# leotimus/recommender-tensorflow

Measured on AMD Instinct MI355X. Metric: examples/sec DeepFM batch=65536 (full train step), higher is better.
Workload: dtype f32 (MLP GEMM operands: fp16 hi+lo split, 3 products, fp32 accumulate)

## Files before the change

include/mi355x_rec.h:

```cpp
#ifndef MI355X_REC_H
#define MI355X_REC_H

#include <stddef.h>
#include <stdint.h>

#ifdef __cplusplus
extern "C" {
#endif

typedef void* mi_stream_t;

enum mi_status {
  MI_OK = 0,
  MI_ERR_INVALID = -1,
  MI_ERR_UNSUPPORTED = -2,
  MI_ERR_LAUNCH = -3,
  MI_ERR_WORKSPACE = -4
};

int32_t mi_abi_version(void);
const char* mi_last_error(void);
const char* mi_build_info(void);

typedef struct mi_step_state {
// ... 100 lines not shown
  float lr_t;
  float decay, momentum;
  float lr_power, l1, l2;
} mi_opt_hparams;

int32_t mi_axpy(float* y, const float* x, int64_t n, float alpha, mi_stream_t stream);

int32_t mi_dense_apply(float* param, float* slot0, float* slot1, const float* grad, int64_t n,
                       const mi_opt_hparams* hp, mi_stream_t stream);

int32_t mi_sparse_apply(float* table, float* t_slot0, float* t_slot1, float* lin_w, float* l_slot0,
                        float* l_slot1, int32_t* last_step, const int32_t* uniq_rows,
                        const int32_t* seg_start, const int32_t* sorted_entry,
                        const int32_t* num_uniq, int64_t n_max, const float* d_rows,
                        const float* d_lin, int32_t E, int32_t step, const mi_opt_hparams* hp,
                        int32_t lin_stride, int64_t table_stride, int64_t grad_stride, mi_stream_t stream);

int32_t mi_sparse_apply_fused(float* table, float* t_slot0, float* t_slot1, float* lin_w, float* l_slot0,
                              float* l_slot1, int32_t* last_step, const int32_t* uniq_rows,
                              const int32_t* seg_start, const int32_t* sorted_entry, const int32_t* num_uniq,
                              int64_t n_max, const float* d_concat, int64_t ld_dconcat, const float* sumv,
                              const float* d_logit_fm, const float* d_logit_lin, int32_t F, int32_t E,
                              int32_t step, const mi_opt_hparams* hp, int32_t lin_stride, int64_t table_stride, mi_stream_t stream);

enum mi_catchup_flags { MI_CATCHUP_DEFER_SLOTS = 1, MI_CATCHUP_BOUNDED = 2, MI_CATCHUP_KEEP_STAMPS = 4, MI_CATCHUP_LOCAL_ORDER = 8 };
int32_t mi_catchup_local_chunk_rows(void);
int32_t mi_catchup_bounded_runs(float beta1, float beta2, float epsilon);
int32_t mi_catchup_local_plan(int64_t n_max, int64_t num_uniq, int64_t* plan);
int32_t mi_catchup_gap_keys(const int32_t* uniq_rows, const int32_t* num_uniq, const int32_t* last_step, int64_t n_max,
                            int32_t step_to, int32_t* keys, int32_t lin_stride, mi_stream_t stream);

int32_t mi_catchup_rows_by_gap(const int32_t* uniq_rows, const int32_t* num_uniq, const int32_t* last_step, int64_t n_max,
                               int32_t step_to, int32_t lin_stride, int32_t* rows_out, void* workspace,
                               size_t workspace_bytes, mi_stream_t stream);


int32_t mi_selftest_sqrt(uint32_t first_bits, int64_t count, uint64_t* mismatches, mi_stream_t stream);

int32_t mi_selftest_div(float d, uint32_t first_bits, int64_t count, uint64_t* out, mi_stream_t stream);

int32_t mi_sparse_catchup(float* table, float* t_m, float* t_v, float* lin_w, float* l_m, float* l_v,
                          int32_t* last_step, const int32_t* uniq_rows, const int32_t* num_uniq,
                          int64_t n_max, int32_t E, int32_t step_to, const float* lr_table,
                          float beta1, float beta2, float epsilon, int32_t flags, int32_t lin_stride,
                          int64_t table_stride, mi_stream_t stream);

// ... 266 lines not shown
```

recommender-tensorflow_amd/csrc/optim.hip:

```cpp
#include "common.h"
#include "optim_rules.h"
#include <algorithm>

namespace {

constexpr int kBlock = 256;

__global__ __launch_bounds__(kBlock) void dense_apply_k(float* __restrict__ w, float* __restrict__ s0,
                                                        float* __restrict__ s1,
                                                        const float* __restrict__ g, int64_t n,
                                                        Hp h, const mi_step_state_t* __restrict__ st) {
  if (st) h.lr_t = st->lr_t;
  const int64_t stride = static_cast<int64_t>(gridDim.x) * kBlock;
  for (int64_t i = static_cast<int64_t>(blockIdx.x) * kBlock + threadIdx.x; i < n; i += stride) {
    float wv = w[i], a = s0 ? s0[i] : 0.f, b = s1 ? s1[i] : 0.f;
    dense_rule(h, wv, a, b, g[i]);
    w[i] = wv;
    if (s0) s0[i] = a;
    if (s1) s1[i] = b;
  }
}

typedef float f32x4_t __attribute__((ext_vector_type(4)));
__device__ __forceinline__ float4 ld4_nt(const float* p) {
// ... 5 lines not shown
  __builtin_nontemporal_store(x, reinterpret_cast<f32x4_t*>(p));
}

struct FusedGrad {
  const float* d_concat; int64_t ldd; const float* sumv; const float* dlf; const float* dll; int F;
  int64_t b0;
};

constexpr int kLongSeg = 48;
constexpr int kRun = 1;

struct ApplyArgs {
  float* table; float* t0; float* t1;
  float* lin_w; float* l0; float* l1;
  int32_t* last_step;
  const int32_t* uniq_rows; const int32_t* seg_start; const int32_t* sorted_entry; const int32_t* num_uniq;
  const float* d_rows; const float* d_lin;
  int E, step;
  float* out_rows; float* out_lin; int u_begin, u_count;
  int ls;
  const mi_step_state_t* st;
  int64_t ts;
  int64_t gs, gls, os, ols;
};

template <bool FUSED>
__device__ __forceinline__ void seg_accumulate(const ApplyArgs& a, const FusedGrad& fg, int k_beg, int k_end, int l,
                                               bool lane_on, const float4& w, float4& g, float& gl) {
  const int E = a.E;
  for (int k = k_beg; k < k_end; ++k) {
    const int64_t e = a.sorted_entry[k];
    if constexpr (FUSED) {
      const int64_t bg = e / fg.F;
      const int f = static_cast<int>(e - bg * fg.F);
      const int64_t b = bg - fg.b0;
      if (a.table && lane_on) {
        float4 v = make_float4(0.f, 0.f, 0.f, 0.f);
        if (fg.d_concat) v = ld4(fg.d_concat + b * fg.ldd + static_cast<int64_t>(f) * E + 4 * l);
        if (fg.dlf) {
          const float gf = fg.dlf[b];
          if (fg.sumv) {
            const float4 sv = ld4(fg.sumv + b * E + 4 * l);
            v.x += gf * (sv.x - w.x); v.y += gf * (sv.y - w.y);
            v.z += gf * (sv.z - w.z); v.w += gf * (sv.w - w.w);
          } else {
            v.x -= gf * w.x; v.y -= gf * w.y; v.z -= gf * w.z; v.w -= gf * w.w;
          }
// ... 58 lines not shown
      for (int j = 0; j < missed; ++j) { s0 = s0 * h.beta1; s1 = s1 * h.beta2; }
      sparse_rule(h, lw, s0, s1, gl);
      a.lin_w[o] = lw;
      if (a.l0) a.l0[o] = s0;
      if (a.l1) a.l1[o] = s1;
    }
    if (a.last_step) a.last_step[r * a.ls] = a.step;
  }
}

__device__ __forceinline__ void store_row(const ApplyArgs& a, int64_t u, int l, bool lane_on, const float4& g, float gl) {
  if (a.out_rows && lane_on) st4(a.out_rows + u * a.os + 4 * l, g);
  if (a.out_lin && l == 0) a.out_lin[u * a.ols] = gl;
}

template <int LPR, bool FUSED, bool STORE = false>
__global__ __launch_bounds__(kBlock) void sparse_apply_k(ApplyArgs a, Hp h, const FusedGrad fg) {
  if (a.st) { a.step = a.st->step; h.lr_t = a.st->lr_t; }
  int64_t u = (static_cast<int64_t>(blockIdx.x) * kBlock + threadIdx.x) / LPR;
  const int l = threadIdx.x & (LPR - 1);
  if (u >= (STORE ? a.u_count : *a.num_uniq)) return;
  if (STORE) u += a.u_begin;
  const int s_beg = a.seg_start[u], s_end = a.seg_start[u + 1];
  if (s_end - s_beg > kLongSeg) return;
  const int64_t r = STORE ? u : static_cast<int64_t>(a.uniq_rows[u]);
  const bool lane_on = 4 * l < a.E;
  float4 g = make_float4(0.f, 0.f, 0.f, 0.f);
  float gl = 0.f;
  float4 w = make_float4(0.f, 0.f, 0.f, 0.f);
  if (a.table && lane_on && (!STORE || fg.dlf)) w = ld4(a.table + r * a.ts + 4 * l);
  RowState q;
  if constexpr (!STORE) q = load_row_state(a, h, r, l, lane_on);
  seg_accumulate<FUSED>(a, fg, s_beg, s_end, l, lane_on, w, g, gl);
  if constexpr (STORE) store_row(a, u, l, lane_on, g, gl);
  else apply_row(a, h, r, l, lane_on, w, g, gl, q);
}

template <int LPR, bool FUSED, bool STORE = false>
__global__ __launch_bounds__(kBlock) void sparse_apply_long_k(ApplyArgs a, Hp h, const FusedGrad fg) {
  if (a.st) { a.step = a.st->step; h.lr_t = a.st->lr_t; }
  constexpr int G = kBlock / LPR;
  __shared__ int list[kBlock];
  __shared__ int n_list;
  __shared__ float4 part[kBlock];
  __shared__ float part_l[G];
  const int U = STORE ? a.u_count : *a.num_uniq;
  const int ub = STORE ? a.u_begin : 0;
  const int t = threadIdx.x, l = t & (LPR - 1), grp = t / LPR;
  const bool lane_on = 4 * l < a.E;
  const int64_t per_round = static_cast<int64_t>(kBlock) * gridDim.x;
  {
    int any = 0;
    for (int64_t base = 0; base < U; base += per_round) {
      const int64_t u = base + (static_cast<int64_t>(t / kRun) * gridDim.x + blockIdx.x) * kRun + t % kRun;
      if (u < U) any |= (a.seg_start[ub + u + 1] - a.seg_start[ub + u] > kLongSeg) ? 1 : 0;
    }
    if (!__syncthreads_or(any)) return;
  }
  for (int64_t base = 0; base < U; base += per_round) {
    if (t == 0) n_list = 0;
    __syncthreads();
    const int64_t u = base + (static_cast<int64_t>(t / kRun) * gridDim.x + blockIdx.x) * kRun + t % kRun;
    if (u < U && a.seg_start[ub + u + 1] - a.seg_start[ub + u] > kLongSeg) list[atomicAdd(&n_list, 1)] = static_cast<int>(ub + u);
    __syncthreads();
    const int n = n_list;
    for (int j = 0; j < n; ++j) {
      const int uu = list[j];
      const int64_t r = STORE ? static_cast<int64_t>(uu) : static_cast<int64_t>(a.uniq_rows[uu]);
      const int s_beg = a.seg_start[uu], s_end = a.seg_start[uu + 1];
      const int per = (s_end - s_beg + G - 1) / G;
      const int k0 = min(s_end, s_beg + grp * per), k1 = min(s_end, k0 + per);
      float4 g = make_float4(0.f, 0.f, 0.f, 0.f);
      float gl = 0.f;
      float4 w = make_float4(0.f, 0.f, 0.f, 0.f);
      if (a.table && lane_on && (!STORE || fg.dlf)) w = ld4(a.table + r * a.ts + 4 * l);
      seg_accumulate<FUSED>(a, fg, k0, k1, l, lane_on, w, g, gl);
      part[t] = g;
      if (l == 0) part_l[grp] = gl;
      __syncthreads();
      if (grp == 0) {
        g = part[l];
        gl = part_l[0];
#pragma unroll 4
        for (int q = 1; q < G; ++q) {
          const float4 v = part[q * LPR + l];
          g.x += v.x; g.y += v.y; g.z += v.z; g.w += v.w;
          gl += part_l[q];
        }
        if constexpr (STORE) store_row(a, uu, l, lane_on, g, gl);
        else apply_row(a, h, r, l, lane_on, w, g, gl, load_row_state(a, h, r, l, lane_on));
      }
      __syncthreads();
    }
  }
}

__device__ __forceinline__ float sqrt_rn_fixup(float x) {
  float s = __builtin_amdgcn_sqrtf(x);
  const float sm = __uint_as_float(__float_as_uint(s) - 1u), sp = __uint_as_float(__float_as_uint(s) + 1u);
  const float rm = fmaf(-sm, s, x), rp = fmaf(-sp, s, x);
  s = (rm <= 0.f) ? sm : s;
  s = (rp > 0.f) ? sp : s;
  return s;
}
__device__ __forceinline__ float sqrt_rn_inrange(float x) {
  const float r = __builtin_amdgcn_rsqf(x);
  float s = x * r, h = 0.5f * r;
  const float e = fmaf(-h, s, 0.5f);
  h = fmaf(h, e, h);
  s = fmaf(s, e, s);
  const float d = fmaf(-s, s, x);
  return fmaf(d, h, s);
}
__device__ __forceinline__ float div_rn_inrange(float n, float d) {
  float r = __builtin_amdgcn_rcpf(d);
  const float e = fmaf(-d, r, 1.0f);
// ... 474 lines not shown
    default: { constexpr int L = 64; CALL; } break; \
  }

static int32_t check_hp(const char* who, const mi_opt_hparams* hp) {
  if (!hp || hp->kind < MI_OPT_ADAM || hp->kind > MI_OPT_SGD) {
    mi::set_error("%s: bad optimizer kind", who);
    return MI_ERR_INVALID;
  }
  if (hp->kind == MI_OPT_FTRL && hp->lr_power != -0.5f) {
    mi::set_error("%s: Ftrl learning_rate_power %f unsupported (TF default -0.5 only)", who, hp->lr_power);
    return MI_ERR_UNSUPPORTED;
  }
  return MI_OK;
}

__global__ __launch_bounds__(kBlock) void axpy_k(float* __restrict__ y, const float* __restrict__ x, int64_t n, float alpha) {
  const int64_t i = static_cast<int64_t>(blockIdx.x) * kBlock + threadIdx.x;
  if (i < n) y[i] = y[i] + alpha * x[i];
}

unsigned long_grid(int64_t n_max) {
  return static_cast<unsigned>(std::min<int64_t>(1024, mi::ceil_div(n_max, kBlock)));
}

__global__ void step_advance_k(mi_step_state_t* __restrict__ st, const float* __restrict__ lr_table) {
  const int s = st->step + 1;
  st->step = s;
  st->lr_t = lr_table ? lr_table[s] : 0.f;
  st->seed_term = static_cast<uint64_t>(s) * 1000003ull;
}

extern "C" {

int32_t mi_step_advance(mi_step_state_t* device_state, const float* lr_table, mi_stream_t stream) {
  MI_REQUIRE(device_state, "step_advance: null state");
  step_advance_k<<<dim3(1), dim3(1), 0, mi::as_stream(stream)>>>(device_state, lr_table);
  MI_CHECK_LAUNCH("step_advance");
  return MI_OK;
}

int32_t mi_axpy(float* y, const float* x, int64_t n, float alpha, mi_stream_t stream) {
  MI_REQUIRE(n >= 0 && (n == 0 || (x && y)), "axpy: n=%lld", (long long)n);
  if (n == 0) return MI_OK;
  axpy_k<<<dim3((unsigned)mi::ceil_div(n, kBlock)), dim3(kBlock), 0, mi::as_stream(stream)>>>(y, x, n, alpha);
  MI_CHECK_LAUNCH("axpy");
  return MI_OK;
}


int32_t mi_dense_apply(float* param, float* slot0, float* slot1, const float* grad, int64_t n,
                       const mi_opt_hparams* hp, mi_stream_t stream) {
  if (int32_t rc = check_hp("dense_apply", hp)) return rc;
  MI_REQUIRE(n >= 0, "dense_apply: n=%lld", (long long)n);
  if (n == 0) return MI_OK;
  MI_REQUIRE(param && grad, "dense_apply: null buffer");
  MI_REQUIRE(hp->kind == MI_OPT_SGD || slot0, "dense_apply: optimizer needs slot0");
  MI_REQUIRE((hp->kind != MI_OPT_ADAM && hp->kind != MI_OPT_FTRL && hp->kind != MI_OPT_RMSPROP) || slot1,
             "dense_apply: optimizer needs slot1");
  int64_t nb = mi::ceil_div(n, kBlock);
  if (nb > 4096) nb = 4096;
  dense_apply_k<<<dim3((unsigned)nb), dim3(kBlock), 0, mi::as_stream(stream)>>>(param, slot0, slot1, grad, n, make_hp(hp), mi::step_state());
  MI_CHECK_LAUNCH("dense_apply");
  return MI_OK;
}

int32_t mi_sparse_apply(float* table, float* t_slot0, float* t_slot1, float* lin_w, float* l_slot0,
                        float* l_slot1, int32_t* last_step, const int32_t* uniq_rows,
                        const int32_t* seg_start, const int32_t* sorted_entry,
                        const int32_t* num_uniq, int64_t n_max, const float* d_rows,
                        const float* d_lin, int32_t E, int32_t step, const mi_opt_hparams* hp,
                        int32_t lin_stride, int64_t table_stride, int64_t grad_stride, mi_stream_t stream) {
  if (int32_t rc = check_hp("sparse_apply", hp)) return rc;
  MI_REQUIRE(grad_stride == 0 || (grad_stride >= (table ? E : 1) && (!table || (grad_stride & 3) == 0)),
             "sparse_apply: grad_stride=%lld (0 = d_rows E apart and d_lin 1 apart, else one record per entry)", (long long)grad_stride);
  if (!table) table_stride = 0;
  MI_REQUIRE(table_stride == 0 || (table_stride >= E && (table_stride & 3) == 0), "%s: table_stride=%lld (0 = E, else >= E and a multiple of 4)", "sparse_apply", (long long)table_stride);
  const int64_t ts = table_stride ? table_stride : E;

  MI_REQUIRE(lin_stride >= 1, "sparse_apply: lin_stride=%d", lin_stride);
  MI_REQUIRE(n_max >= 0, "sparse_apply: n_max=%lld", (long long)n_max);
  if (n_max == 0) return MI_OK;
  MI_REQUIRE(table || lin_w, "sparse_apply: nothing to update");
  MI_REQUIRE(uniq_rows && seg_start && sorted_entry && num_uniq, "sparse_apply: null index buffer");
  MI_REQUIRE(!table || (d_rows && E >= 4 && E <= 256 && (E & 3) == 0 && mi::aligned16(table) && mi::aligned16(d_rows)),
             "sparse_apply: table needs d_rows, E multiple of 4 in [4,256], 16-byte alignment");
  MI_REQUIRE(!lin_w || d_lin, "sparse_apply: lin_w needs d_lin");
  const bool need0 = hp->kind != MI_OPT_SGD;
  const bool need1 = hp->kind == MI_OPT_ADAM || hp->kind == MI_OPT_FTRL || hp->kind == MI_OPT_RMSPROP;
  MI_REQUIRE(!table || ((!need0 || t_slot0) && (!need1 || t_slot1)), "sparse_apply: table slots missing");
  MI_REQUIRE(!lin_w || ((!need0 || l_slot0) && (!need1 || l_slot1)), "sparse_apply: linear slots missing");
  const int lpr = table ? lanes_per_row(E) : 1;
  const int64_t blocks = mi::ceil_div(n_max * lpr, kBlock);
  MI_REQUIRE(blocks <= INT32_MAX, "sparse_apply: grid too large");
  const Hp h = make_hp(hp);
  ApplyArgs a{table, t_slot0, t_slot1, lin_w, l_slot0, l_slot1, last_step, uniq_rows, seg_start, sorted_entry,
              num_uniq, d_rows, d_lin, E, step};
  a.ls = lin_stride; a.ts = ts;
  a.gs = grad_stride ? grad_stride : E; a.gls = grad_stride ? grad_stride : 1;
  a.st = mi::step_state();
  MI_DISPATCH_LPR(lpr, (sparse_apply_k<L, false><<<dim3((unsigned)blocks), dim3(kBlock), 0, mi::as_stream(stream)>>>(
                           a, h, FusedGrad{})));
  MI_CHECK_LAUNCH("sparse_apply");
  if (n_max > kLongSeg) {
    MI_DISPATCH_LPR(lpr, (sparse_apply_long_k<L, false><<<dim3(long_grid(n_max)), dim3(kBlock), 0, mi::as_stream(stream)>>>(
                             a, h, FusedGrad{})));
    MI_CHECK_LAUNCH("sparse_apply(long segments)");
  }
  return MI_OK;
}

int32_t mi_sparse_apply_fused(float* table, float* t_slot0, float* t_slot1, float* lin_w, float* l_slot0,
                              float* l_slot1, int32_t* last_step, const int32_t* uniq_rows,
                              const int32_t* seg_start, const int32_t* sorted_entry, const int32_t* num_uniq,
                              int64_t n_max, const float* d_concat, int64_t ld_dconcat, const float* sumv,
                              const float* d_logit_fm, const float* d_logit_lin, int32_t F, int32_t E,
                              int32_t step, const mi_opt_hparams* hp, int32_t lin_stride, int64_t table_stride, mi_stream_t stream) {
  if (int32_t rc = check_hp("sparse_apply_fused", hp)) return rc;
  if (!table) table_stride = 0;
  MI_REQUIRE(table_stride == 0 || (table_stride >= E && (table_stride & 3) == 0), "%s: table_stride=%lld (0 = E, else >= E and a multiple of 4)", "sparse_apply_fused", (long long)table_stride);
  const int64_t ts = table_stride ? table_stride : E;

  MI_REQUIRE(lin_stride >= 1, "sparse_apply_fused: lin_stride=%d", lin_stride);
  MI_REQUIRE(n_max >= 0 && F > 0, "sparse_apply_fused: n_max=%lld F=%d", (long long)n_max, F);
  if (n_max == 0) return MI_OK;
  MI_REQUIRE(table || lin_w, "sparse_apply_fused: nothing to update");
  MI_REQUIRE(uniq_rows && seg_start && sorted_entry && num_uniq, "sparse_apply_fused: null index buffer");
  MI_REQUIRE(!table || (E >= 4 && E <= 256 && (E & 3) == 0 && mi::aligned16(table)),
             "sparse_apply_fused: E multiple of 4 in [4,256], 16-byte alignment");
  MI_REQUIRE(!table || d_concat || d_logit_fm, "sparse_apply_fused: table update needs d_concat and/or d_logit_fm");
  MI_REQUIRE(!d_concat || (ld_dconcat >= (int64_t)F * E && (ld_dconcat & 3) == 0 && mi::aligned16(d_concat)),
             "sparse_apply_fused: d_concat leading dimension / alignment");
  MI_REQUIRE(!d_logit_fm || (sumv ? mi::aligned16(sumv) : d_concat != nullptr),
             "sparse_apply_fused: FM gradient needs sumv, or a d_concat that already carries d_logit_fm * sumv");
  MI_REQUIRE(!lin_w || d_logit_lin, "sparse_apply_fused: lin_w needs d_logit_lin");
  const bool need0 = hp->kind != MI_OPT_SGD;
  const bool need1 = hp->kind == MI_OPT_ADAM || hp->kind == MI_OPT_FTRL || hp->kind == MI_OPT_RMSPROP;
  MI_REQUIRE(!table || ((!need0 || t_slot0) && (!need1 || t_slot1)), "sparse_apply_fused: table slots missing");
  MI_REQUIRE(!lin_w || ((!need0 || l_slot0) && (!need1 || l_slot1)), "sparse_apply_fused: linear slots missing");
  const int lpr = table ? lanes_per_row(E) : 1;
  const int64_t blocks = mi::ceil_div(n_max * lpr, kBlock);
  MI_REQUIRE(blocks <= INT32_MAX, "sparse_apply_fused: grid too large");
  const Hp h = make_hp(hp);
  const FusedGrad fg{d_concat, ld_dconcat, sumv, d_logit_fm, d_logit_lin, F, 0};
  ApplyArgs a{table, t_slot0, t_slot1, lin_w, l_slot0, l_slot1, last_step, uniq_rows, seg_start, sorted_entry,
              num_uniq, nullptr, nullptr, E, step};
  a.ls = lin_stride; a.ts = ts;
  a.st = mi::step_state();
  MI_DISPATCH_LPR(lpr, (sparse_apply_k<L, true><<<dim3((unsigned)blocks), dim3(kBlock), 0, mi::as_stream(stream)>>>(a, h, fg)));
  MI_CHECK_LAUNCH("sparse_apply_fused");
  if (n_max > kLongSeg) {
    MI_DISPATCH_LPR(lpr, (sparse_apply_long_k<L, true><<<dim3(long_grid(n_max)), dim3(kBlock), 0, mi::as_stream(stream)>>>(a, h, fg)));
    MI_CHECK_LAUNCH("sparse_apply_fused(long segments)");
  }
  return MI_OK;
}

int32_t mi_entry_grads_segsum(const float* rows, const int32_t* seg_start, const int32_t* sorted_entry, int64_t u_begin,
                              int64_t u_count, const float* d_concat, int64_t ld_dconcat, const float* sumv,
                              const float* d_logit_fm, const float* d_logit_lin, int64_t b0, int32_t F, int32_t E,
                              float* out_rows, float* out_lin, int64_t out_row0, int64_t rows_stride, int64_t out_stride,
                              mi_stream_t stream) {
  MI_REQUIRE(rows_stride == 0 || (rows_stride >= E && (rows_stride & 3) == 0), "entry_grads_segsum: rows_stride=%lld", (long long)rows_stride);
  MI_REQUIRE(out_stride == 0 || (out_stride >= (out_rows ? E : 1) && (!out_rows || (out_stride & 3) == 0)),
             "entry_grads_segsum: out_stride=%lld (0 = out_rows E apart and out_lin 1 apart, else one record per request)", (long long)out_stride);
  MI_REQUIRE(u_begin >= 0 && u_count >= 0 && u_begin + u_count <= INT32_MAX && F > 0 && b0 >= 0, "entry_grads_segsum: u_begin=%lld u_count=%lld",
             (long long)u_begin, (long long)u_count);
  MI_REQUIRE(out_row0 >= 0 && out_row0 <= u_begin, "entry_grads_segsum: out_row0=%lld must lie in [0, u_begin=%lld]", (long long)out_row0,
             (long long)u_begin);
  if (u_count == 0) return MI_OK;
  MI_REQUIRE(seg_start && sorted_entry && (out_rows || out_lin), "entry_grads_segsum: null buffer");
  MI_REQUIRE(!out_rows || (E >= 4 && E <= 256 && (E & 3) == 0 && mi::aligned16(out_rows) && (d_concat || d_logit_fm)),
             "entry_grads_segsum: row gradients need E multiple of 4 in [4,256] and d_concat and/or d_logit_fm");
  MI_REQUIRE(!d_concat || (ld_dconcat >= (int64_t)F * E && (ld_dconcat & 3) == 0 && mi::aligned16(d_concat)),
             "entry_grads_segsum: d_concat leading dimension / alignment");
  MI_REQUIRE(!d_logit_fm || (sumv && rows && mi::aligned16(sumv) && mi::aligned16(rows)), "entry_grads_segsum: the FM gradient needs sumv and the rows");
  MI_REQUIRE(!out_lin || d_logit_lin, "entry_grads_segsum: out_lin needs d_logit_lin");
  const int lpr = out_rows ? lanes_per_row(E) : 1;
// ... 124 lines not shown
```

recommender-tensorflow_amd/mi355x_rec/_lib.py:

```python
import ctypes as C
import os

import torch

_HERE = os.path.dirname(os.path.abspath(__file__))
LIB_PATH = os.path.join(_HERE, "libmi355x_rec.so")

ABI_VERSION = 21


class MiError(RuntimeError):
    pass


class OptHparams(C.Structure):
    _fields_ = [("kind", C.c_int32), ("lr", C.c_float), ("beta1", C.c_float), ("beta2", C.c_float),
                ("epsilon", C.c_float), ("lr_t", C.c_float), ("decay", C.c_float),
                ("momentum", C.c_float), ("lr_power", C.c_float), ("l1", C.c_float),
                ("l2", C.c_float)]


AMAX_SLOTS = 64
MAX_WEIGHT_JOBS = 8

# ... 91 lines not shown
    "mi_numeric_raw_bwd_workspace_bytes": (_sz, [_i64, _i32]),
    "mi_numeric_raw_bwd": (_i32, [_p, _p, _i64, _i32, _p, _p, _sz, _p]),
    "mi_embed_fm_linear_bwd": (_i32, [_p, _i64, _p, _i64, _p, _p, _p, _p, _p, _i64, _i32, _i32, _p, _p, _p]),
    "mi_entry_grads_segsum": (_i32, [_p, _p, _p, _i64, _i64, _p, _i64, _p, _p, _p, _i64, _i32, _i32, _p, _p, _i64, _i64, _i64, _p]),
    "mi_numeric_embed_bwd_workspace_bytes": (_sz, [_i64, _i32, _i32]),
    "mi_numeric_embed_bwd": (_i32, [_p, _p, _i64, _p, _i64, _i64, _p, _p, _p, _i64, _i32, _i32, _p,
                                    _p, _p, _sz, _p]),
    "mi_sort_unique_workspace_bytes": (_sz, [_i64]),
    "mi_sort_unique_fields_workspace_bytes": (_sz, [_i64, _i32]),
    "mi_sort_unique_fields": (_i32, [_p, _p, _i64, _i32, _i64, _p, _p, _p, _p, _p, _sz, _i32, _p]),
    "mi_sort_unique_rows": (_i32, [_p, _i64, _i64, _p, _p, _p, _p, _p, _sz, _p]),
    "mi_sort_unique_rows_slots": (_i32, [_p, _i64, _i64, _p, _p, _p, _p, _p, _p, _sz, _p]),
    "mi_global_rows": (_i32, [_p, _p, _i64, _i32, _p, _p]),
    "mi_shard_keys": (_i32, [_p, _i64, _i32, _i64, _i64, _i32, _p, _p]),
    "mi_route_requests": (_i32, [_p, _p, _i64, _i64, _i32, _p, _p, _p]),
    "mi_segment_slots": (_i32, [_p, _p, _p, _i64, _p, _p]),
    "mi_axpy": (_i32, [_p, _p, _i64, _f32, _p]),
    "mi_gather_u32": (_i32, [_p, _p, _i64, _p, _p]),
    "mi_dense_apply": (_i32, [_p, _p, _p, _p, _i64, C.POINTER(OptHparams), _p]),
    "mi_sparse_apply": (_i32, [_p, _p, _p, _p, _p, _p, _p, _p, _p, _p, _p, _i64, _p, _p, _i32, _i32,
                               C.POINTER(OptHparams), _i32, _i64, _i64, _p]),
    "mi_sparse_apply_fused": (_i32, [_p, _p, _p, _p, _p, _p, _p, _p, _p, _p, _p, _i64, _p, _i64, _p, _p, _p, _i32,
                                     _i32, _i32, C.POINTER(OptHparams), _i32, _i64, _p]),
    "mi_dense_fwd_gathered": (_i32, [_p, _p, _p, _i32, _i32, _p, _p, _p, _i64, _i64, _i32, _i32, _f32, _u64, _amax, _i64, _p]),
    "mi_dense_bwd_weight_gathered": (_i32, [_p, _p, _p, _i32, _i32, _p, _i64, _p, _p, _i64, _i32, _p, _sz, _amax, _i64, _p]),
    "mi_selftest_sqrt": (_i32, [_u32, _i64, _p, _p]),
    "mi_selftest_div": (_i32, [_f32, _u32, _i64, _p, _p]),
    "mi_catchup_gap_keys": (_i32, [_p, _p, _p, _i64, _i32, _p, _i32, _p]),
    "mi_catchup_rows_by_gap": (_i32, [_p, _p, _p, _i64, _i32, _i32, _p, _p, _sz, _p]),
    "mi_catchup_local_chunk_rows": (_i32, []),
    "mi_catchup_local_plan": (_i32, [_i64, _i64, _p]),
    "mi_catchup_bounded_runs": (_i32, [_f32, _f32, _f32]),
    "mi_sparse_catchup": (_i32, [_p, _p, _p, _p, _p, _p, _p, _p, _p, _i64, _i32, _i32, _p, _f32, _f32,
                                 _f32, _i32, _i32, _i64, _p]),
    "mi_set_gemm_mode": (_i32, [_i32]),
    "mi_absmax": (_i32, [_p, _i64, _p, _p]),
    "mi_get_gemm_mode": (_i32, []),
    "mi_dense_fwd": (_i32, [_p, _i64, _p, _p, _p, _i64, _i64, _i32, _i32, _i32, _f32, _u64, _amax, _p]),
    "mi_dense_bwd_data": (_i32, [_p, _i64, _p, _p, _i64, _p, _i64, _i64, _i32, _i32, _f32, _i32, _amax, _p]),
    "mi_dense_bwd_weight_workspace_bytes": (_sz, [_i64, _i32, _i32]),
    "mi_dense_bwd_data_vec_planes": (_i32, [_p, _i64, _p, _p, _i64, _f32, _p, _i64, _pl, _i64, _i32, _p, _p, _i64, _p]),
    "mi_dense_bwd_weight_planes_workspace_bytes": (_sz, [_i64, _i32, _i32]),
    "mi_dense_bwd_weight_planes": (_i32, [_p, _p, _p, _p, _i64, _i32, _i32, _p, _sz, _p, _p]),
    "mi_dense_bwd_weight": (_i32, [_p, _i64, _p, _i64, _p, _p, _i64, _i32, _i32, _p, _sz, _amax, _p]),
    "mi_dense_bwd_weight_planes_batch_workspace_bytes": (_sz, [_p, _i32, _i64]),
    "mi_dense_bwd_weight_planes_batch": (_i32, [_p, _i32, _i64, _p, _sz, _p]),
# ... 107 lines not shown
```

recommender-tensorflow_amd/mi355x_rec/engine.py:

```python
import ctypes as C
import json
import os
import math

import numpy as np
import torch

from . import _lib
from ._lib import OptHparams, check, ptr

OPT_KINDS = {"Adam": 0, "Adagrad": 1, "Ftrl": 2, "RMSProp": 3, "SGD": 4}


def _align(n, a=16):
    return (n + a - 1) // a * a


def predict_buffers(B, device):
    cls = torch.empty(B, 1, dtype=torch.int64, device=device)
    return {"logits": torch.empty(B, 1, dtype=torch.float32, device=device),
            "logistic": torch.empty(B, 1, dtype=torch.float32, device=device),
            "probabilities": torch.empty(B, 2, dtype=torch.float32, device=device), "class_ids": cls, "classes": cls}


# ... 182 lines not shown
    others = [s for (d, _), ss in _SIDE_STREAMS.items() if d == key[0] for s in ss]
    seen, fallback = set(), None
    while len(found) <= k:
        pick = None
        for _ in range(32):
            s = torch.cuda.Stream(device=device, priority=prio)
            if s.cuda_stream in seen or any(s.cuda_stream == o.cuda_stream for o in others + [main]):
                continue
            seen.add(s.cuda_stream)
            if not _streams_overlap(main, s, cyc):
                continue
            if fallback is None:
                fallback = s
            if all(_streams_overlap(o, s, cyc) for o in others):
                pick = s
                break
        pick = pick or fallback or torch.cuda.Stream(device=device, priority=prio)
        found.append(pick)
        others.append(pick)
        fallback = None
    return found[k]

class DeepFM:

    def __init__(self, vocab_sizes, n_numeric=0, embedding_size=4, hidden_units=(16, 16),
                 use_linear=True, use_mf=True, use_dnn=True, dropout=0.0, optimizer=None,
                 linear_optimizer=None, reduction="mean", device="cuda", seed=0, shard=None,
                 gemm="f16x2", numeric="embed", activation="relu", catchup="bounded", field_dims=None, wide_fields=None,
                 deep_numeric=None, wide_numeric=None, _kernels=None):
        if len(vocab_sizes) + n_numeric == 0:
            raise ValueError("At least 1 feature column of categorical_columns or numeric_columns "
                             "must be specified.")
        if not (use_linear or use_mf or use_dnn):
            raise ValueError("At least 1 of linear, mf or dnn component must be used.")
        acts = {"relu": 1, None: 0, "identity": 0, "linear": 0, "sigmoid": 2, "tanh": 3}
        name = activation if (activation is None or isinstance(activation, str)) else getattr(activation, "__name__", None)
        if name not in acts:
            raise NotImplementedError("activation %r: the GEMM epilogues implement relu, sigmoid, tanh and identity" % (activation,))
        self.act = acts[name]
        if numeric not in ("embed", "raw"):
            raise ValueError("numeric must be 'embed' or 'raw'")
        if numeric == "raw" and use_mf:
            raise ValueError("raw numeric columns belong to the canned estimators, which have no FM term")
        if catchup not in ("exact", "bounded"):
            raise ValueError("catchup must be 'exact' or 'bounded'")
        self.field_dims = None if field_dims is None else [int(d) for d in field_dims]
# ... 306 lines not shown
        else:
            out.update(table=None if self.table is None else self.table.cpu().numpy(),
                       lin_w_local=None if self.lin_w is None else self.lin_w.cpu().numpy())
        if self.num_emb_off is not None:
            out["num_emb"] = self._seg(self.dense, self.num_emb_off, (self.n_numeric, self.E)).cpu().numpy()
        if self.lin_num_off is not None:
            out["lin_num"] = self._seg(self.dense, self.lin_num_off, (self.n_numeric,)).cpu().numpy()
        return out

    def _buf(self, name, shape, dtype=torch.float32):
        n = int(np.prod(shape))
        cur = self._ws.get(name)
        if cur is None or cur.numel() < n or cur.dtype != dtype:
            cur = torch.empty(max(n, 1), dtype=dtype, device=self.device)
            self._ws[name] = cur
            self._alloc_gen += 1
        return cur[:n].view(*shape)

    def _bytes(self, name, nbytes):
        n = (int(nbytes) + 255) // 256 * 256 + 256
        cur = self._ws.get(name)
        if cur is None or cur.numel() < n:
            cur = torch.empty(n, dtype=torch.uint8, device=self.device)
            self._ws[name] = cur
            self._alloc_gen += 1
        return cur

    def _planes(self, name, rows, K):
        cur = self._pl.get(name)
        if cur is None or cur.rows < rows or cur.K != K:
            cur = self._pl[name] = PlaneBuf(self.k, rows, K, self.device)
            self._alloc_gen += 1
        return cur.struct

    def _av(self, name):
        i = self._amax_idx.setdefault(name, len(self._amax_idx))
        return self._amax[i * _lib.AMAX_SLOTS:(i + 1) * _lib.AMAX_SLOTS]

    def _ga(self, a, b, out):
        if self.gemm != "f16x2":
            return None
        p = lambda n: None if n is None else ptr(self._av(n))
        return _lib.GemmAmax(p(a), p(b), p(out))

    def _split_weights(self, train, amax=None):
        hidden = self.layers[:-1]
# ... 940 lines not shown
        lin_lr_t = self.lin_sched.lr_t(step) if self.lin_sched else 0.0
        if self._frozen is not None:
            self.d_grad.index_fill_(0, self._frozen, 0.0)
        if self.lin_opt is None:
            if self.P:
                k.mi_dense_apply(self.dense, self.d_s0, self.d_s1, self.d_grad, self.P, hp)
            sparse_hp = [(True, True, hp)]
        else:
            lhp = self.lin_opt.hparams(lin_lr_t)
            if self.wide_off:
                k.mi_dense_apply(self.dense, self.d_s0, self.d_s1, self.d_grad, self.wide_off, hp)
            o = self.wide_off
            sl = lambda t: t[o:] if t is not None else None
            k.mi_dense_apply(self.dense[o:], sl(self.dl_s0), sl(self.dl_s1), self.d_grad[o:], self.P - o, lhp)
            sparse_hp = [(True, False, hp), (False, True, lhp)]
        if n_max > 0:
            for do_table, do_lin, h in sparse_hp:
                tb = self.table if (do_table and self.use_emb) else None
                lw = self.lin_w if (do_lin and self.use_linear) else None
                if tb is None and lw is None:
                    continue
                slots = (tb, self.t_s0 if tb is not None else None, self.t_s1 if tb is not None else None,
                         lw, self.l_s0 if lw is not None else None, self.l_s1 if lw is not None else None)
                if fused is not None:
                    d_concat, sumv, dlogit = fused
                    k.mi_sparse_apply_fused(*slots, self.last_step, uniq, seg, sorted_entry, num_uniq, n_max,
                                            d_concat if tb is not None else None, self.D,
                                            sumv if (tb is not None and self.use_mf) else None,
                                            dlogit if (tb is not None and self.use_mf) else None,
                                            dlogit if lw is not None else None, self.F, self.E, step, h, self.ls, self.ts)
                else:
                    k.mi_sparse_apply(*slots, self.last_step, uniq, seg, sorted_entry, num_uniq, n_max,
                                      d_rows if tb is not None else None, d_lin if lw is not None else None, self.E,
                                      step, h, self.ls, self.ts, 0)
        self.step = step

    def graph_ok(self):
        return (self.shard is None and self.device.type == "cuda" and
                not (self.sched is not None and self.lin_sched is not None and self.sched is not self.lin_sched))

    def graph_train_step(self, ids, labels, x_num=None):
        if self.shard is not None or self.device.type != "cuda":
            raise NotImplementedError("graph_train_step: single-GPU models")
        if not self.graph_ok():
            raise NotImplementedError("graph_train_step: the device-resident step state carries ONE lr_t (two different Adams)")
        self._prep(ids, labels, x_num)
        graphs = self.__dict__.setdefault("_graphs", {})
        shape = tuple(ids.shape)
        g = self._graph = graphs.get(shape)
        if g is not None and g["gen"] != self._graph_gen():
            graphs.clear()
            g = self._graph = None
            self._warm_shapes().add(shape)
        if g is None:
            warm = self._warm_shapes()
            if shape not in warm:
                warm.add(shape)
# ... 295 lines not shown
```

Before: 25.40 million.

## Record long segments in a workspace list instead of rescanning all unique rows

```diff
diff --git a/include/mi355x_rec.h b/include/mi355x_rec.h
--- a/include/mi355x_rec.h
+++ b/include/mi355x_rec.h
@@ -146,6 +146,22 @@
                               int64_t n_max, const float* d_concat, int64_t ld_dconcat, const float* sumv,
                               const float* d_logit_fm, const float* d_logit_lin, int32_t F, int32_t E,
                               int32_t step, const mi_opt_hparams* hp, int32_t lin_stride, int64_t table_stride, mi_stream_t stream);
+
+size_t mi_sparse_apply_workspace_bytes(int64_t n_max);
+int32_t mi_sparse_apply_ws(float* table, float* t_slot0, float* t_slot1, float* lin_w, float* l_slot0,
+                           float* l_slot1, int32_t* last_step, const int32_t* uniq_rows,
+                           const int32_t* seg_start, const int32_t* sorted_entry,
+                           const int32_t* num_uniq, int64_t n_max, const float* d_rows,
+                           const float* d_lin, int32_t E, int32_t step, const mi_opt_hparams* hp,
+                           int32_t lin_stride, int64_t table_stride, int64_t grad_stride, void* workspace,
+                           size_t workspace_bytes, mi_stream_t stream);
+int32_t mi_sparse_apply_fused_ws(float* table, float* t_slot0, float* t_slot1, float* lin_w, float* l_slot0,
+                                 float* l_slot1, int32_t* last_step, const int32_t* uniq_rows,
+                                 const int32_t* seg_start, const int32_t* sorted_entry, const int32_t* num_uniq,
+                                 int64_t n_max, const float* d_concat, int64_t ld_dconcat, const float* sumv,
+                                 const float* d_logit_fm, const float* d_logit_lin, int32_t F, int32_t E,
+                                 int32_t step, const mi_opt_hparams* hp, int32_t lin_stride, int64_t table_stride,
+                                 void* workspace, size_t workspace_bytes, mi_stream_t stream);
 
 enum mi_catchup_flags { MI_CATCHUP_DEFER_SLOTS = 1, MI_CATCHUP_BOUNDED = 2, MI_CATCHUP_KEEP_STAMPS = 4, MI_CATCHUP_LOCAL_ORDER = 8 };
 int32_t mi_catchup_local_chunk_rows(void);
diff --git a/recommender-tensorflow_amd/csrc/optim.hip b/recommender-tensorflow_amd/csrc/optim.hip
--- a/recommender-tensorflow_amd/csrc/optim.hip
+++ b/recommender-tensorflow_amd/csrc/optim.hip
@@ -51,7 +51,9 @@
   const mi_step_state_t* st;
   int64_t ts;
   int64_t gs, gls, os, ols;
+  int32_t* long_ws; int long_cap;
 };
+constexpr int kLongWsHead = 4;
 
 template <bool FUSED>
 __device__ __forceinline__ void seg_accumulate(const ApplyArgs& a, const FusedGrad& fg, int k_beg, int k_end, int l,
@@ -156,7 +158,13 @@
   if (u >= (STORE ? a.u_count : *a.num_uniq)) return;
   if (STORE) u += a.u_begin;
   const int s_beg = a.seg_start[u], s_end = a.seg_start[u + 1];
-  if (s_end - s_beg > kLongSeg) return;
+  if (s_end - s_beg > kLongSeg) {
+    if (a.long_ws && l == 0) {
+      const int at = atomicAdd(a.long_ws, 1);
+      if (at < a.long_cap) a.long_ws[kLongWsHead + at] = static_cast<int>(u);
+    }
+    return;
+  }
   const int64_t r = STORE ? u : static_cast<int64_t>(a.uniq_rows[u]);
   const bool lane_on = 4 * l < a.E;
   float4 g = make_float4(0.f, 0.f, 0.f, 0.f);
@@ -170,18 +178,61 @@
   else apply_row(a, h, r, l, lane_on, w, g, gl, q);
 }
 
+template <int LPR, bool FUSED, bool STORE>
+__device__ __forceinline__ void long_row(const ApplyArgs& a, const Hp& h, const FusedGrad& fg, int uu, float4* part, float* part_l) {
+  constexpr int G = kBlock / LPR;
+  const int t = threadIdx.x, l = t & (LPR - 1), grp = t / LPR;
+  const bool lane_on = 4 * l < a.E;
+  const int64_t r = STORE ? static_cast<int64_t>(uu) : static_cast<int64_t>(a.uniq_rows[uu]);
+  const int s_beg = a.seg_start[uu], s_end = a.seg_start[uu + 1];
+  const int per = (s_end - s_beg + G - 1) / G;
+  const int k0 = min(s_end, s_beg + grp * per), k1 = min(s_end, k0 + per);
+  float4 g = make_float4(0.f, 0.f, 0.f, 0.f);
+  float gl = 0.f;
+  float4 w = make_float4(0.f, 0.f, 0.f, 0.f);
+  if (a.table && lane_on && (!STORE || fg.dlf)) w = ld4(a.table + r * a.ts + 4 * l);
+  seg_accumulate<FUSED>(a, fg, k0, k1, l, lane_on, w, g, gl);
+  part[t] = g;
+  if (l == 0) part_l[grp] = gl;
+  __syncthreads();
+  if (grp == 0) {
+    g = part[l];
+    gl = part_l[0];
+#pragma unroll 4
+    for (int q = 1; q < G; ++q) {
+      const float4 v = part[q * LPR + l];
+      g.x += v.x; g.y += v.y; g.z += v.z; g.w += v.w;
+      gl += part_l[q];
+    }
+    if constexpr (STORE) store_row(a, uu, l, lane_on, g, gl);
+    else apply_row(a, h, r, l, lane_on, w, g, gl, load_row_state(a, h, r, l, lane_on));
+  }
+  __syncthreads();
+}
+
 template <int LPR, bool FUSED, bool STORE = false>
 __global__ __launch_bounds__(kBlock) void sparse_apply_long_k(ApplyArgs a, Hp h, const FusedGrad fg) {
   if (a.st) { a.step = a.st->step; h.lr_t = a.st->lr_t; }
-  constexpr int G = kBlock / LPR;
   __shared__ int list[kBlock];
   __shared__ int n_list;
   __shared__ float4 part[kBlock];
-  __shared__ float part_l[G];
+  __shared__ float part_l[kBlock / LPR];
+  const int t = threadIdx.x;
+  if (a.long_ws) {
+    if (t == 0) n_list = min(__hip_atomic_load(a.long_ws, __ATOMIC_RELAXED, __HIP_MEMORY_SCOPE_AGENT), a.long_cap);
+    __syncthreads();
+    const int n = n_list;
+    if (n == 0) return;
+    for (int j = blockIdx.x; j < n; j += gridDim.x)
+      long_row<LPR, FUSED, STORE>(a, h, fg, __hip_atomic_load(a.long_ws + kLongWsHead + j, __ATOMIC_RELAXED, __HIP_MEMORY_SCOPE_AGENT), part, part_l);
+    if (t == 0 && atomicAdd(a.long_ws + 1, 1) == static_cast<int>(gridDim.x) - 1) {
+      __hip_atomic_store(a.long_ws, 0, __ATOMIC_RELAXED, __HIP_MEMORY_SCOPE_AGENT);
+      __hip_atomic_store(a.long_ws + 1, 0, __ATOMIC_RELAXED, __HIP_MEMORY_SCOPE_AGENT);
+    }
+    return;
+  }
   const int U = STORE ? a.u_count : *a.num_uniq;
   const int ub = STORE ? a.u_begin : 0;
-  const int t = threadIdx.x, l = t & (LPR - 1), grp = t / LPR;
-  const bool lane_on = 4 * l < a.E;
   const int64_t per_round = static_cast<int64_t>(kBlock) * gridDim.x;
   {
     int any = 0;
@@ -198,34 +249,7 @@
     if (u < U && a.seg_start[ub + u + 1] - a.seg_start[ub + u] > kLongSeg) list[atomicAdd(&n_list, 1)] = static_cast<int>(ub + u);
     __syncthreads();
     const int n = n_list;
-    for (int j = 0; j < n; ++j) {
-      const int uu = list[j];
-      const int64_t r = STORE ? static_cast<int64_t>(uu) : static_cast<int64_t>(a.uniq_rows[uu]);
-      const int s_beg = a.seg_start[uu], s_end = a.seg_start[uu + 1];
-      const int per = (s_end - s_beg + G - 1) / G;
-      const int k0 = min(s_end, s_beg + grp * per), k1 = min(s_end, k0 + per);
-      float4 g = make_float4(0.f, 0.f, 0.f, 0.f);
-      float gl = 0.f;
-      float4 w = make_float4(0.f, 0.f, 0.f, 0.f);
-      if (a.table && lane_on && (!STORE || fg.dlf)) w = ld4(a.table + r * a.ts + 4 * l);
-      seg_accumulate<FUSED>(a, fg, k0, k1, l, lane_on, w, g, gl);
-      part[t] = g;
-      if (l == 0) part_l[grp] = gl;
-      __syncthreads();
-      if (grp == 0) {
-        g = part[l];
-        gl = part_l[0];
-#pragma unroll 4
-        for (int q = 1; q < G; ++q) {
-          const float4 v = part[q * LPR + l];
-          g.x += v.x; g.y += v.y; g.z += v.z; g.w += v.w;
-          gl += part_l[q];
-        }
-        if constexpr (STORE) store_row(a, uu, l, lane_on, g, gl);
-        else apply_row(a, h, r, l, lane_on, w, g, gl, load_row_state(a, h, r, l, lane_on));
-      }
-      __syncthreads();
-    }
+    for (int j = 0; j < n; ++j) long_row<LPR, FUSED, STORE>(a, h, fg, list[j], part, part_l);
   }
 }
 
@@ -746,54 +770,30 @@
 unsigned long_grid(int64_t n_max) {
   return static_cast<unsigned>(std::min<int64_t>(1024, mi::ceil_div(n_max, kBlock)));
 }
-
-__global__ void step_advance_k(mi_step_state_t* __restrict__ st, const float* __restrict__ lr_table) {
-  const int s = st->step + 1;
-  st->step = s;
-  st->lr_t = lr_table ? lr_table[s] : 0.f;
-  st->seed_term = static_cast<uint64_t>(s) * 1000003ull;
-}
-
-extern "C" {
-
-int32_t mi_step_advance(mi_step_state_t* device_state, const float* lr_table, mi_stream_t stream) {
-  MI_REQUIRE(device_state, "step_advance: null state");
-  step_advance_k<<<dim3(1), dim3(1), 0, mi::as_stream(stream)>>>(device_state, lr_table);
-  MI_CHECK_LAUNCH("step_advance");
+static unsigned long_grid(int64_t n_max, const ApplyArgs& a) {
+  return a.long_ws ? std::max(1u, std::min(long_grid(n_max), static_cast<unsigned>(a.long_cap))) : long_grid(n_max);
+}
+
+static int64_t long_cap(int64_t n_max) { return n_max / (kLongSeg + 1); }
+
+static int32_t long_list(ApplyArgs& a, const char* who, int64_t n_max, void* workspace, size_t workspace_bytes) {
+  a.long_ws = nullptr; a.long_cap = 0;
+  if (!workspace) return MI_OK;
+  const int64_t cap = long_cap(n_max);
+  MI_REQUIRE(cap <= INT32_MAX - kLongWsHead && workspace_bytes >= (kLongWsHead + static_cast<size_t>(cap)) * sizeof(int32_t) &&
+                 (reinterpret_cast<uintptr_t>(workspace) & 3) == 0,
+             "%s: workspace of %zu bytes (mi_sparse_apply_workspace_bytes, 4-byte aligned)", who, workspace_bytes);
+  a.long_ws = static_cast<int32_t*>(workspace); a.long_cap = static_cast<int>(cap);
   return MI_OK;
 }
 
-int32_t mi_axpy(float* y, const float* x, int64_t n, float alpha, mi_stream_t stream) {
-  MI_REQUIRE(n >= 0 && (n == 0 || (x && y)), "axpy: n=%lld", (long long)n);
-  if (n == 0) return MI_OK;
-  axpy_k<<<dim3((unsigned)mi::ceil_div(n, kBlock)), dim3(kBlock), 0, mi::as_stream(stream)>>>(y, x, n, alpha);
-  MI_CHECK_LAUNCH("axpy");
-  return MI_OK;
-}
-
-
-int32_t mi_dense_apply(float* param, float* slot0, float* slot1, const float* grad, int64_t n,
-                       const mi_opt_hparams* hp, mi_stream_t stream) {
-  if (int32_t rc = check_hp("dense_apply", hp)) return rc;
-  MI_REQUIRE(n >= 0, "dense_apply: n=%lld", (long long)n);
-  if (n == 0) return MI_OK;
-  MI_REQUIRE(param && grad, "dense_apply: null buffer");
-  MI_REQUIRE(hp->kind == MI_OPT_SGD || slot0, "dense_apply: optimizer needs slot0");
-  MI_REQUIRE((hp->kind != MI_OPT_ADAM && hp->kind != MI_OPT_FTRL && hp->kind != MI_OPT_RMSPROP) || slot1,
-             "dense_apply: optimizer needs slot1");
-  int64_t nb = mi::ceil_div(n, kBlock);
-  if (nb > 4096) nb = 4096;
-  dense_apply_k<<<dim3((unsigned)nb), dim3(kBlock), 0, mi::as_stream(stream)>>>(param, slot0, slot1, grad, n, make_hp(hp), mi::step_state());
-  MI_CHECK_LAUNCH("dense_apply");
-  return MI_OK;
-}
-
-int32_t mi_sparse_apply(float* table, float* t_slot0, float* t_slot1, float* lin_w, float* l_slot0,
+static int32_t sparse_apply_impl(float* table, float* t_slot0, float* t_slot1, float* lin_w, float* l_slot0,
                         float* l_slot1, int32_t* last_step, const int32_t* uniq_rows,
                         const int32_t* seg_start, const int32_t* sorted_entry,
                         const int32_t* num_uniq, int64_t n_max, const float* d_rows,
                         const float* d_lin, int32_t E, int32_t step, const mi_opt_hparams* hp,
-                        int32_t lin_stride, int64_t table_stride, int64_t grad_stride, mi_stream_t stream) {
+                        int32_t lin_stride, int64_t table_stride, int64_t grad_stride, void* workspace, size_t workspace_bytes,
+                        mi_stream_t stream) {
   if (int32_t rc = check_hp("sparse_apply", hp)) return rc;
   MI_REQUIRE(grad_stride == 0 || (grad_stride >= (table ? E : 1) && (!table || (grad_stride & 3) == 0)),
              "sparse_apply: grad_stride=%lld (0 = d_rows E apart and d_lin 1 apart, else one record per entry)", (long long)grad_stride);
@@ -822,23 +822,25 @@
   a.ls = lin_stride; a.ts = ts;
   a.gs = grad_stride ? grad_stride : E; a.gls = grad_stride ? grad_stride : 1;
   a.st = mi::step_state();
+  if (int32_t rc = long_list(a, "sparse_apply", n_max, workspace, workspace_bytes)) return rc;
   MI_DISPATCH_LPR(lpr, (sparse_apply_k<L, false><<<dim3((unsigned)blocks), dim3(kBlock), 0, mi::as_stream(stream)>>>(
                            a, h, FusedGrad{})));
   MI_CHECK_LAUNCH("sparse_apply");
   if (n_max > kLongSeg) {
-    MI_DISPATCH_LPR(lpr, (sparse_apply_long_k<L, false><<<dim3(long_grid(n_max)), dim3(kBlock), 0, mi::as_stream(stream)>>>(
+    MI_DISPATCH_LPR(lpr, (sparse_apply_long_k<L, false><<<dim3(long_grid(n_max, a)), dim3(kBlock), 0, mi::as_stream(stream)>>>(
                              a, h, FusedGrad{})));
     MI_CHECK_LAUNCH("sparse_apply(long segments)");
   }
   return MI_OK;
 }
 
-int32_t mi_sparse_apply_fused(float* table, float* t_slot0, float* t_slot1, float* lin_w, float* l_slot0,
+static int32_t sparse_apply_fused_impl(float* table, float* t_slot0, float* t_slot1, float* lin_w, float* l_slot0,
                               float* l_slot1, int32_t* last_step, const int32_t* uniq_rows,
                               const int32_t* seg_start, const int32_t* sorted_entry, const int32_t* num_uniq,
                               int64_t n_max, const float* d_concat, int64_t ld_dconcat, const float* sumv,
                               const float* d_logit_fm, const float* d_logit_lin, int32_t F, int32_t E,
-                              int32_t step, const mi_opt_hparams* hp, int32_t lin_stride, int64_t table_stride, mi_stream_t stream) {
+                              int32_t step, const mi_opt_hparams* hp, int32_t lin_stride, int64_t table_stride, void* workspace,
+                              size_t workspace_bytes, mi_stream_t stream) {
   if (int32_t rc = check_hp("sparse_apply_fused", hp)) return rc;
   if (!table) table_stride = 0;
   MI_REQUIRE(table_stride == 0 || (table_stride >= E && (table_stride & 3) == 0), "%s: table_stride=%lld (0 = E, else >= E and a multiple of 4)", "sparse_apply_fused", (long long)table_stride);
@@ -870,13 +872,105 @@
               num_uniq, nullptr, nullptr, E, step};
   a.ls = lin_stride; a.ts = ts;
   a.st = mi::step_state();
+  if (int32_t rc = long_list(a, "sparse_apply_fused", n_max, workspace, workspace_bytes)) return rc;
   MI_DISPATCH_LPR(lpr, (sparse_apply_k<L, true><<<dim3((unsigned)blocks), dim3(kBlock), 0, mi::as_stream(stream)>>>(a, h, fg)));
   MI_CHECK_LAUNCH("sparse_apply_fused");
   if (n_max > kLongSeg) {
-    MI_DISPATCH_LPR(lpr, (sparse_apply_long_k<L, true><<<dim3(long_grid(n_max)), dim3(kBlock), 0, mi::as_stream(stream)>>>(a, h, fg)));
+    MI_DISPATCH_LPR(lpr, (sparse_apply_long_k<L, true><<<dim3(long_grid(n_max, a)), dim3(kBlock), 0, mi::as_stream(stream)>>>(a, h, fg)));
     MI_CHECK_LAUNCH("sparse_apply_fused(long segments)");
   }
   return MI_OK;
+}
+
+__global__ void step_advance_k(mi_step_state_t* __restrict__ st, const float* __restrict__ lr_table) {
+  const int s = st->step + 1;
+  st->step = s;
+  st->lr_t = lr_table ? lr_table[s] : 0.f;
+  st->seed_term = static_cast<uint64_t>(s) * 1000003ull;
+}
+
+extern "C" {
+
+int32_t mi_step_advance(mi_step_state_t* device_state, const float* lr_table, mi_stream_t stream) {
+  MI_REQUIRE(device_state, "step_advance: null state");
+  step_advance_k<<<dim3(1), dim3(1), 0, mi::as_stream(stream)>>>(device_state, lr_table);
+  MI_CHECK_LAUNCH("step_advance");
+  return MI_OK;
+}
+
+int32_t mi_axpy(float* y, const float* x, int64_t n, float alpha, mi_stream_t stream) {
+  MI_REQUIRE(n >= 0 && (n == 0 || (x && y)), "axpy: n=%lld", (long long)n);
+  if (n == 0) return MI_OK;
+  axpy_k<<<dim3((unsigned)mi::ceil_div(n, kBlock)), dim3(kBlock), 0, mi::as_stream(stream)>>>(y, x, n, alpha);
+  MI_CHECK_LAUNCH("axpy");
+  return MI_OK;
+}
+
+
+int32_t mi_dense_apply(float* param, float* slot0, float* slot1, const float* grad, int64_t n,
+                       const mi_opt_hparams* hp, mi_stream_t stream) {
+  if (int32_t rc = check_hp("dense_apply", hp)) return rc;
+  MI_REQUIRE(n >= 0, "dense_apply: n=%lld", (long long)n);
+  if (n == 0) return MI_OK;
+  MI_REQUIRE(param && grad, "dense_apply: null buffer");
+  MI_REQUIRE(hp->kind == MI_OPT_SGD || slot0, "dense_apply: optimizer needs slot0");
+  MI_REQUIRE((hp->kind != MI_OPT_ADAM && hp->kind != MI_OPT_FTRL && hp->kind != MI_OPT_RMSPROP) || slot1,
+             "dense_apply: optimizer needs slot1");
+  int64_t nb = mi::ceil_div(n, kBlock);
+  if (nb > 4096) nb = 4096;
+  dense_apply_k<<<dim3((unsigned)nb), dim3(kBlock), 0, mi::as_stream(stream)>>>(param, slot0, slot1, grad, n, make_hp(hp), mi::step_state());
+  MI_CHECK_LAUNCH("dense_apply");
+  return MI_OK;
+}
+
+int32_t mi_sparse_apply(float* table, float* t_slot0, float* t_slot1, float* lin_w, float* l_slot0,
+                        float* l_slot1, int32_t* last_step, const int32_t* uniq_rows,
+                        const int32_t* seg_start, const int32_t* sorted_entry,
+                        const int32_t* num_uniq, int64_t n_max, const float* d_rows,
+                        const float* d_lin, int32_t E, int32_t step, const mi_opt_hparams* hp,
+                        int32_t lin_stride, int64_t table_stride, int64_t grad_stride, mi_stream_t stream) {
+  return sparse_apply_impl(table, t_slot0, t_slot1, lin_w, l_slot0, l_slot1, last_step, uniq_rows, seg_start, sorted_entry, num_uniq,
+                           n_max, d_rows, d_lin, E, step, hp, lin_stride, table_stride, grad_stride, nullptr, 0, stream);
+}
+
+int32_t mi_sparse_apply_ws(float* table, float* t_slot0, float* t_slot1, float* lin_w, float* l_slot0,
+                           float* l_slot1, int32_t* last_step, const int32_t* uniq_rows,
+                           const int32_t* seg_start, const int32_t* sorted_entry,
+                           const int32_t* num_uniq, int64_t n_max, const float* d_rows,
+                           const float* d_lin, int32_t E, int32_t step, const mi_opt_hparams* hp,
+                           int32_t lin_stride, int64_t table_stride, int64_t grad_stride, void* workspace,
+                           size_t workspace_bytes, mi_stream_t stream) {
+  MI_REQUIRE(workspace, "sparse_apply_ws: null workspace");
+  return sparse_apply_impl(table, t_slot0, t_slot1, lin_w, l_slot0, l_slot1, last_step, uniq_rows, seg_start, sorted_entry, num_uniq,
+                           n_max, d_rows, d_lin, E, step, hp, lin_stride, table_stride, grad_stride, workspace, workspace_bytes, stream);
+}
+
+int32_t mi_sparse_apply_fused(float* table, float* t_slot0, float* t_slot1, float* lin_w, float* l_slot0,
+                              float* l_slot1, int32_t* last_step, const int32_t* uniq_rows,
+                              const int32_t* seg_start, const int32_t* sorted_entry, const int32_t* num_uniq,
+                              int64_t n_max, const float* d_concat, int64_t ld_dconcat, const float* sumv,
+                              const float* d_logit_fm, const float* d_logit_lin, int32_t F, int32_t E,
+                              int32_t step, const mi_opt_hparams* hp, int32_t lin_stride, int64_t table_stride, mi_stream_t stream) {
+  return sparse_apply_fused_impl(table, t_slot0, t_slot1, lin_w, l_slot0, l_slot1, last_step, uniq_rows, seg_start, sorted_entry,
+                                 num_uniq, n_max, d_concat, ld_dconcat, sumv, d_logit_fm, d_logit_lin, F, E, step, hp, lin_stride,
+                                 table_stride, nullptr, 0, stream);
+}
+
+int32_t mi_sparse_apply_fused_ws(float* table, float* t_slot0, float* t_slot1, float* lin_w, float* l_slot0,
+                                 float* l_slot1, int32_t* last_step, const int32_t* uniq_rows,
+                                 const int32_t* seg_start, const int32_t* sorted_entry, const int32_t* num_uniq,
+                                 int64_t n_max, const float* d_concat, int64_t ld_dconcat, const float* sumv,
+                                 const float* d_logit_fm, const float* d_logit_lin, int32_t F, int32_t E,
+                                 int32_t step, const mi_opt_hparams* hp, int32_t lin_stride, int64_t table_stride,
+                                 void* workspace, size_t workspace_bytes, mi_stream_t stream) {
+  MI_REQUIRE(workspace, "sparse_apply_fused_ws: null workspace");
+  return sparse_apply_fused_impl(table, t_slot0, t_slot1, lin_w, l_slot0, l_slot1, last_step, uniq_rows, seg_start, sorted_entry,
+                                 num_uniq, n_max, d_concat, ld_dconcat, sumv, d_logit_fm, d_logit_lin, F, E, step, hp, lin_stride,
+                                 table_stride, workspace, workspace_bytes, stream);
+}
+
+size_t mi_sparse_apply_workspace_bytes(int64_t n_max) {
+  return n_max < 0 ? 0 : (kLongWsHead + static_cast<size_t>(long_cap(n_max))) * sizeof(int32_t);
 }
 
 int32_t mi_entry_grads_segsum(const float* rows, const int32_t* seg_start, const int32_t* sorted_entry, int64_t u_begin,
diff --git a/recommender-tensorflow_amd/mi355x_rec/_lib.py b/recommender-tensorflow_amd/mi355x_rec/_lib.py
--- a/recommender-tensorflow_amd/mi355x_rec/_lib.py
+++ b/recommender-tensorflow_amd/mi355x_rec/_lib.py
@@ -137,6 +137,11 @@
                                C.POINTER(OptHparams), _i32, _i64, _i64, _p]),
     "mi_sparse_apply_fused": (_i32, [_p, _p, _p, _p, _p, _p, _p, _p, _p, _p, _p, _i64, _p, _i64, _p, _p, _p, _i32,
                                      _i32, _i32, C.POINTER(OptHparams), _i32, _i64, _p]),
+    "mi_sparse_apply_workspace_bytes": (_sz, [_i64]),
+    "mi_sparse_apply_ws": (_i32, [_p, _p, _p, _p, _p, _p, _p, _p, _p, _p, _p, _i64, _p, _p, _i32, _i32,
+                                  C.POINTER(OptHparams), _i32, _i64, _i64, _p, _sz, _p]),
+    "mi_sparse_apply_fused_ws": (_i32, [_p, _p, _p, _p, _p, _p, _p, _p, _p, _p, _p, _i64, _p, _i64, _p, _p, _p, _i32,
+                                        _i32, _i32, C.POINTER(OptHparams), _i32, _i64, _p, _sz, _p]),
     "mi_dense_fwd_gathered": (_i32, [_p, _p, _p, _i32, _i32, _p, _p, _p, _i64, _i64, _i32, _i32, _f32, _u64, _amax, _i64, _p]),
     "mi_dense_bwd_weight_gathered": (_i32, [_p, _p, _p, _i32, _i32, _p, _i64, _p, _p, _i64, _i32, _p, _sz, _amax, _i64, _p]),
     "mi_selftest_sqrt": (_i32, [_u32, _i64, _p, _p]),
diff --git a/recommender-tensorflow_amd/mi355x_rec/engine.py b/recommender-tensorflow_amd/mi355x_rec/engine.py
--- a/recommender-tensorflow_amd/mi355x_rec/engine.py
+++ b/recommender-tensorflow_amd/mi355x_rec/engine.py
@@ -228,6 +228,8 @@
     return found[k]
 
 class DeepFM:
+
+    long_list = 1
 
     def __init__(self, vocab_sizes, n_numeric=0, embedding_size=4, hidden_units=(16, 16),
                  use_linear=True, use_mf=True, use_dnn=True, dropout=0.0, optimizer=None,
@@ -580,6 +582,14 @@
         cur = self._ws.get(name)
         if cur is None or cur.numel() < n:
             cur = torch.empty(n, dtype=torch.uint8, device=self.device)
+            self._ws[name] = cur
+            self._alloc_gen += 1
+        return cur
+
+    def _zeros(self, name, nbytes):
+        cur = self._ws.get(name)
+        if cur is None or cur.numel() < int(nbytes):
+            cur = torch.zeros((int(nbytes) + 255) // 256 * 256 + 256, dtype=torch.uint8, device=self.device)
             self._ws[name] = cur
             self._alloc_gen += 1
         return cur
@@ -1566,17 +1576,23 @@
                     continue
                 slots = (tb, self.t_s0 if tb is not None else None, self.t_s1 if tb is not None else None,
                          lw, self.l_s0 if lw is not None else None, self.l_s1 if lw is not None else None)
+                ws = ()
+                if self.long_list and self.shard is None and hasattr(k, "mi_sparse_apply_fused_ws"):
+                    lws = self._zeros("long_ws", k.query("mi_sparse_apply_workspace_bytes", n_max))
+                    ws = (lws, lws.numel())
                 if fused is not None:
                     d_concat, sumv, dlogit = fused
-                    k.mi_sparse_apply_fused(*slots, self.last_step, uniq, seg, sorted_entry, num_uniq, n_max,
-                                            d_concat if tb is not None else None, self.D,
-                                            sumv if (tb is not None and self.use_mf) else None,
-                                            dlogit if (tb is not None and self.use_mf) else None,
-                                            dlogit if lw is not None else None, self.F, self.E, step, h, self.ls, self.ts)
+                    (k.mi_sparse_apply_fused_ws if ws else k.mi_sparse_apply_fused)(
+                        *slots, self.last_step, uniq, seg, sorted_entry, num_uniq, n_max,
+                        d_concat if tb is not None else None, self.D,
+                        sumv if (tb is not None and self.use_mf) else None,
+                        dlogit if (tb is not None and self.use_mf) else None,
+                        dlogit if lw is not None else None, self.F, self.E, step, h, self.ls, self.ts, *ws)
                 else:
-                    k.mi_sparse_apply(*slots, self.last_step, uniq, seg, sorted_entry, num_uniq, n_max,
-                                      d_rows if tb is not None else None, d_lin if lw is not None else None, self.E,
-                                      step, h, self.ls, self.ts, 0)
+                    (k.mi_sparse_apply_ws if ws else k.mi_sparse_apply)(
+                        *slots, self.last_step, uniq, seg, sorted_entry, num_uniq, n_max,
+                        d_rows if tb is not None else None, d_lin if lw is not None else None, self.E,
+                        step, h, self.ls, self.ts, 0, *ws)
         self.step = step
 
     def graph_ok(self):
```

After: 25.43 million, median of 2. No clear change (+0.1%).
